# yixuan/spectra

Measured on AMD Instinct MI355X. Metric: eigenpairs_per_sec, higher is better.
Workload: dtype f64

## Files before the change

include/mispec.h:

```cpp
#ifndef MISPEC_H
#define MISPEC_H

#include <stdint.h>

#ifdef __cplusplus
extern "C" {
#endif

#define MISPEC_OK 0
#define MISPEC_EINVAL (-1)
#define MISPEC_ELOGIC (-2)
#define MISPEC_ERUNTIME (-3)

typedef struct mispec_ctx mispec_ctx;
typedef struct mispec_csr mispec_csr;
typedef struct mispec_fac mispec_fac;

const char* mispec_last_error(void);
const char* mispec_version(void);

int mispec_set_option(const char* name, const char* value);
const char* mispec_get_option(const char* name);

int mispec_ctx_create(int device, void* hip_stream, mispec_ctx** out);
// ... 32 lines not shown
int64_t mispec_csr_rows(const mispec_csr* A);
int64_t mispec_csr_cols(const mispec_csr* A);
int64_t mispec_csr_local_rows(const mispec_csr* A);
int64_t mispec_csr_local_nnz(const mispec_csr* A);
int mispec_csr_offset_codes(const mispec_csr* A);
int mispec_csr_use_offset_codes(mispec_csr* A, int enable);
int mispec_csr_use_windows(mispec_csr* A, int enable);
int mispec_csr_windows_info(const mispec_csr* A, int64_t* blocks, int64_t* covered_entries, int64_t* lds_doubles);
int mispec_csr_windows_in_use(const mispec_csr* A);
int mispec_csr_windows_table(const mispec_csr* A, int32_t* records_out, int64_t capacity);
int mispec_csr_windows_host(int64_t n_rows, int64_t n_cols, int64_t row_begin, const int32_t* rowptr, const int32_t* colind,
                            int32_t* records_out);
int mispec_csr_spmv_format(const mispec_csr* A);
int mispec_csr_set_spmv_format(mispec_csr* A, int format);
double mispec_csr_spmv_bytes(const mispec_csr* A, int stored);
int mispec_csr_coeff(const mispec_csr* A, int64_t i, int64_t j, double* out);
int mispec_csr_download(const mispec_csr* A, int32_t* rowptr_host, int32_t* colind_host, double* val_host);

int mispec_spmv(const mispec_csr* A, const double* x_dev, double* y_dev);
int mispec_spmv_host(const mispec_csr* A, const double* x_host, double* y_host);
int mispec_spmm_host(const mispec_csr* A, const double* X_host, int64_t ldx, int k, double* Y_host, int64_t ldy);
int mispec_spmm(const mispec_csr* A, const double* X_dev, int64_t ldx, int k, double* Y_dev, int64_t ldy);
int mispec_spmm_plan(int k, int forced_panel, int* widths_out, int cap, int* count);
int mispec_csr_reorder(mispec_csr* A, int method, int* applied);
int mispec_csr_reordering(const mispec_csr* A, double* far_before, double* far_after);
int mispec_csr_permutation(const mispec_csr* A, int32_t* perm_out);
int mispec_csr_tiles_info(const mispec_csr* A, int64_t* segments, int64_t* entries, int64_t* padding, int64_t* chunks);
int mispec_csr_staged_info(const mispec_csr* A, int64_t* bins, int64_t* slots, int64_t* batches, int64_t* chunks);
int mispec_last_ingest_info(double* seconds_out, int count);
int mispec_ingest_threads(void);
// ... 184 lines not shown
```

spectra_amd/__init__.py:

```python
import ctypes as C
import enum
import os

import numpy as np

from . import _capi
from ._capi import MispecError, Profile, build_library, check, lib

__all__ = ["SortRule", "CompInfo", "Context", "SparseSymMatProd", "SparseGenMatProd", "SparseSymShiftSolve", "SymEigsSolver",
           "SymEigsShiftSolver", "GenEigsSolver", "SVDMatOp", "PartialSVDSolver", "SparseRegularInverse", "SparseCholesky", "SymGEigsSolver", "SymShiftInvert", "SymGEigsShiftSolver", "SparseGenRealShiftSolve", "GenEigsRealShiftSolver", "shard_block",
           "Factorization", "tridiag_qr", "tridiag_eigen", "hess_qr", "double_shift_qr", "hess_schur", "hess_eigen", "MispecError", "build_library", "shard_range", "BAND_OFFSETS", "SYNTH_SEED",
           "SparseHermMatProd", "DenseHermMatProd", "HermEigsSolver", "spmm_plan"]

BAND_OFFSETS = (1, 2, 3, 1000, 1001, 100000, 100001)
SYNTH_SEED = 20240607


ORTH_MODES = {"reference": 0, "onesweep": 1, "onesweep-eager": 1 | 0x100, "onesweep-recorrect": 1 | 0x200, "onesweep-restart-check": 1 | 0x400,
              "onesweep-onered": 1 | 0x800, "onesweep-twored": 1 | 0x1000, "onesweep-onered-eager": 1 | 0x800 | 0x100}


def _orth_mode_value(mode):
    if isinstance(mode, str):
        if mode not in ORTH_MODES:
            raise ValueError("unknown orthogonalisation mode %r: one of %s" % (mode, ", ".join(sorted(ORTH_MODES))))
        return ORTH_MODES[mode]
    if isinstance(mode, int) and mode in ORTH_MODES.values():
# ... 165 lines not shown


def get_option(name):
    v = lib().mispec_get_option(name.encode())
    return None if v is None else v.decode()


def spmm_plan(k, panel=0):
    cap = max(int(k), 1)
    out = (C.c_int * cap)()
    count = C.c_int(0)
    check(lib().mispec_spmm_plan(int(k), int(panel), out, cap, C.byref(count)))
    return [out[i] for i in range(count.value)]


def default_context():
    global _default_ctx
    if _default_ctx is None:
        _default_ctx = Context(0)
    return _default_ctx


class _DeviceMatrix:

    def __init__(self, ctx, handle):
        self.ctx = ctx
        self.h = handle

    def rows(self):
        return lib().mispec_csr_rows(self.h)
# ... 49 lines not shown
        return 12.0 * self.nnz() + 4.0 * (self.local_rows() + 1) + 8.0 * self.cols() + 8.0 * self.local_rows()

    def offset_codes(self):
        return int(lib().mispec_csr_offset_codes(self.h))

    def use_offset_codes(self, enable=True):
        check(lib().mispec_csr_use_offset_codes(self.h, 1 if enable else 0))

    def use_windows(self, enable=True):
        check(lib().mispec_csr_use_windows(self.h, -1 if enable is None else (1 if enable else 0)))

    def windows_info(self):
        a, b, c = C.c_int64(0), C.c_int64(0), C.c_int64(0)
        check(lib().mispec_csr_windows_info(self.h, C.byref(a), C.byref(b), C.byref(c)))
        return {"blocks": a.value, "covered_entries": b.value, "lds_doubles": c.value}

    def windows_in_use(self):
        return bool(lib().mispec_csr_windows_in_use(self.h))

    def windows_table(self):
        nb = (self.local_rows() + 255) // 256
        out = np.empty((nb, 32), dtype=np.int32)
        check(lib().mispec_csr_windows_table(self.h, _ip(out), out.size))
        return out

    def spmv_format(self):
        return int(lib().mispec_csr_spmv_format(self.h))

    def set_spmv_format(self, fmt=-1):
        check(lib().mispec_csr_set_spmv_format(self.h, int(fmt)))
# ... 1401 lines not shown
```

spectra_amd/_capi.py:

```python
import ctypes as C
import os
import subprocess

_PKG = os.path.dirname(os.path.abspath(__file__))
LIB_PATH = os.path.join(_PKG, "libmispec.so")
EXTRAS_LIB_PATH = os.path.join(_PKG, "libmispec_extras.so")
EXTRAS_PREFIXES = ("mispec_davidson_", "mispec_zdense_", "mispec_zfac_", "mispec_zcsr_", "mispec_hermeigs_")
CSRC = os.path.join(_PKG, "csrc")

MISPEC_OK, MISPEC_EINVAL, MISPEC_ELOGIC, MISPEC_ERUNTIME = 0, -1, -2, -3


class MispecError(RuntimeError):
    """HIP / RCCL failure or a failed small decomposition (std::runtime_error in the C++ API)."""


def build_library(force=False, verbose=False):
    cmd = ["make", "-C", CSRC, "-j8"] + (["-B"] if force else [])
    out = subprocess.run(cmd, stdout=subprocess.PIPE, stderr=subprocess.STDOUT, text=True)
    if verbose or out.returncode != 0:
        print(out.stdout)
    if out.returncode != 0:
        raise RuntimeError("building libmispec.so failed")
    return LIB_PATH
# ... 51 lines not shown
    "mispec_csr_destroy": (C.c_int, [_vp]),
    "mispec_csr_rows": (C.c_int64, [_vp]),
    "mispec_csr_cols": (C.c_int64, [_vp]),
    "mispec_csr_local_rows": (C.c_int64, [_vp]),
    "mispec_csr_local_nnz": (C.c_int64, [_vp]),
    "mispec_csr_offset_codes": (C.c_int, [_vp]),
    "mispec_csr_use_offset_codes": (C.c_int, [_vp, C.c_int]),
    "mispec_csr_use_windows": (C.c_int, [_vp, C.c_int]),
    "mispec_csr_windows_info": (C.c_int, [_vp, _lp, _lp, _lp]),
    "mispec_csr_windows_table": (C.c_int, [_vp, _ip, C.c_int64]),
    "mispec_csr_windows_in_use": (C.c_int, [_vp]),
    "mispec_csr_windows_host": (C.c_int, [C.c_int64, C.c_int64, C.c_int64, _ip, _ip, _ip]),
    "mispec_csr_spmv_format": (C.c_int, [_vp]),
    "mispec_csr_set_spmv_format": (C.c_int, [_vp, C.c_int]),
    "mispec_csr_spmv_bytes": (C.c_double, [_vp, C.c_int]),
    "mispec_csr_coeff": (C.c_int, [_vp, C.c_int64, C.c_int64, _dp]),
    "mispec_csr_download": (C.c_int, [_vp, _ip, _ip, _dp]),
    "mispec_spmv": (C.c_int, [_vp, _vp, _vp]),
    "mispec_spmv_host": (C.c_int, [_vp, _dp, _dp]),
    "mispec_spmm_host": (C.c_int, [_vp, _dp, C.c_int64, C.c_int, _dp, C.c_int64]),
    "mispec_spmv_time": (C.c_int, [_vp, _vp, _vp, C.c_int, C.POINTER(C.c_float)]),
    "mispec_spmm": (C.c_int, [_vp, _vp, C.c_int64, C.c_int, _vp, C.c_int64]),
    "mispec_spmm_time": (C.c_int, [_vp, _vp, C.c_int64, C.c_int, _vp, C.c_int64, C.c_int, C.POINTER(C.c_float)]),
    "mispec_spmm_plan": (C.c_int, [C.c_int, C.c_int, C.POINTER(C.c_int), C.c_int, C.POINTER(C.c_int)]),
    "mispec_symshift_level_plan": (C.c_int, [C.c_int64, C.c_int64, C.c_int, _lp, _lp, _lp, _lp]),
    "mispec_symshift_create": (C.c_int, [_vp, C.c_int64, _ip, _ip, _dp, C.c_char, C.c_int, _vpp]),
    "mispec_symshift_destroy": (C.c_int, [_vp]),
    "mispec_symshift_rows": (C.c_int64, [_vp]),
    "mispec_symshift_bandwidth": (C.c_int, [_vp, _lp, _lp, C.POINTER(C.c_int)]),
    "mispec_csr_tiles_info": (C.c_int, [_vp, _lp, _lp, _lp, _lp]),
# ... 225 lines not shown
```

spectra_amd/csrc/common.hpp:

```cpp
#pragma once

#include <hip/hip_runtime.h>

#include <cstdint>
#include <cstdio>
#include <cstdlib>
#include <new>
#include <functional>
#include <utility>
#include <stdexcept>
#include <string>
#include <vector>

#include "../../include/mispec.h"
#include "../../include/mispec_extras.h"

namespace mispec {

struct Error : std::runtime_error
{
    int code;
    Error(int c, const std::string& m) : std::runtime_error(m), code(c) {}
};

// ... 96 lines not shown
    void alloc(size_t count)
    {
        if (p)
            (void) hipHostFree(p);
        p = nullptr;
        MISPEC_HIP(hipHostMalloc(reinterpret_cast<void**>(&p), count * sizeof(T), hipHostMallocDefault));
        n = count;
    }
};

inline int64_t round_up(int64_t x, int64_t m) { return (x + m - 1) / m * m; }

enum class Opt
{
    orth, one_reduction, orth_kernel, host_turn, small, restart_sync, host_steps, overlap, csr_win, spec_corr, exchange, reorder,
    spmv_staged, spmv_tiles, spmm, host_threads, shift, count
};
enum class Orth { onesweep, onesweep_eager, reference };
enum class OrthKernel { dma, dma2, reg, unset };
enum class HostTurn { fast, copy };
enum class Small { host, host_serial, device };
enum class Exchange { allgather, halo, unset };
enum class Reorder { automatic, rcm, none };
enum class Tri { automatic, off, on };
enum class Spmm { automatic, off, w2, w4, w8 };
int option_choice(Opt o);
template <typename E>
E option_choice(Opt o, E unset)
{
    const int i = option_choice(o);
    return i < 0 ? unset : E(i);
}
bool option_flag(Opt o, bool unset);
int option_int(Opt o, int unset);
struct ShiftOptions
{
    int lds = 1;
    int batch = 0;
    int lanes = 0;
// ... 65 lines not shown
```

spectra_amd/csrc/csr.hip:

```cpp
#include "csr_kernels.hpp"
#include "reorder.hpp"

#include <hip/hip_ext.h>

#include <chrono>

#include <algorithm>
#include <cstdlib>
#include <cstring>
#include <memory>
#include <numeric>

using namespace mispec;

namespace {

template <bool EPI, bool NT, int kThreads, bool CODES, int ITERS = 4>
__global__ __launch_bounds__(kThreads) void k_spmv_csr_stream(const int32_t* __restrict__ rowptr,
                                                               const int32_t* __restrict__ colind,
                                                               const double* __restrict__ val,
                                                               const double* __restrict__ x, double* __restrict__ y,
                                                               int64_t nrows, int nblocks, SpmvEpilogue epi, SpmvCodes cd)
{
    constexpr int kLoadIters = ITERS;
// ... 531 lines not shown
    std::vector<int32_t> rp, ci;
    std::vector<double> v;
    permute_csr(n, rowptr, colind, val, perm, rp, ci, v);
    std::unique_ptr<mispec_csr> B(upload_rows(A.ctx, n, n, rp.data(), ci.data(), v.data(), false, A.structurally_symmetric));
    A.rowptr.swap(B->rowptr);
    A.colind.swap(B->colind);
    A.val.swap(B->val);
    A.codes.swap(B->codes);
    A.dict.swap(B->dict);
    A.dia.swap(B->dia);
    A.dia_off.swap(B->dia_off);
    std::swap(A.ndict, B->ndict);
    std::swap(A.dia_ld, B->dia_ld);
    std::swap(A.ndia, B->ndia);
    std::swap(A.dia_win, B->dia_win);
    A.tiles.swap(B->tiles);
    A.staged.swap(B->staged);
    A.wtab.swap(B->wtab);
    std::swap(A.win_lds_doubles, B->win_lds_doubles);
    std::swap(A.win_covered, B->win_covered);
    std::swap(A.win_blocks, B->win_blocks);
    A.nnz = B->nnz;
    A.perm.alloc(size_t(n));
    MISPEC_HIP(hipMemcpy(A.perm.p, perm.data(), size_t(n) * sizeof(int32_t), hipMemcpyHostToDevice));
    A.perm_host.swap(perm);
    A.inv_host.swap(inv);
    A.reorder_method = 1;
    A.far_before = before;
    A.far_after = after;
    return true;
// ... 859 lines not shown
```

spectra_amd/csrc/csr.hpp:

```cpp
#pragma once
#include <vector>

#include "common.hpp"
#include "tiles.hpp"
#include "staged.hpp"

struct mispec_dia_windows
{
    int nc = 0;
    int total = 0;
    int start[8];
    int len[8];
    int base[8];
    int idx[32];
};

struct mispec_csr
{
    mispec_ctx* ctx = nullptr;
    int64_t n_rows = 0;
    int64_t n_cols = 0;
    int64_t row_begin = 0;
    int64_t row_end = 0;
    int64_t nnz = 0;
    mispec::DevBuf<int32_t> rowptr;
    mispec::DevBuf<int32_t> colind;
    mispec::DevBuf<double> val;
    mispec::DevBuf<uint8_t> codes;
    mispec::DevBuf<int32_t> dict;
    int ndict = 0;
    bool use_codes = true;
    mispec::DevBuf<double> dia;
    mispec::DevBuf<int32_t> dia_off;
    int64_t dia_ld = 0;
    int ndia = 0;
    mispec_dia_windows dia_win;
    mispec::DevBuf<int32_t> wtab;
    int win_lds_doubles = 0;
    int64_t win_covered = 0;
    int64_t win_blocks = 0;
    int use_windows = -1;
    bool windows_active() const
    {
        if (wtab.p == nullptr || win_lds_doubles <= 0 || use_windows == 0)
            return false;
        return use_windows == 1 || double(nnz) >= 9.0 * double(local_rows());
    }
    int forced_format = -1;
    mispec::DevTiles tiles;
    mispec::DevStaged staged;
    mispec::DevBuf<int32_t> perm;
// ... 3 lines not shown
    bool structurally_symmetric = false;
    mutable mispec::DevBuf<double> perm_x, perm_y;
    bool reordered() const { return perm.p != nullptr; }
    mutable mispec::DevBuf<double> stage_x, stage_y;
    mutable mispec::DevBuf<double> spmm_x;

    int64_t local_rows() const { return row_end - row_begin; }
    double algorithmic_bytes() const
    {
        return 12.0 * double(nnz) + 4.0 * double(local_rows() + 1) + 8.0 * double(n_cols) + 8.0 * double(local_rows());
    }
    int spmv_format() const;
    double stored_bytes_for(int format) const
    {
        if (format == 2)
            return 8.0 * double(ndia) * double(local_rows()) + 8.0 * double(n_cols) + 8.0 * double(local_rows());
        if (format == 4)
            return staged.stored_bytes(local_rows(), n_cols);
        if (format == 3)
            return 12.0 * double(tiles.entries) + 8.0 * double(tiles.nchunks) + 12.0 * double(tiles.nseg) + 8.0 * double(n_cols) +
                   8.0 * double(local_rows());
        const double per_entry = format == 1 ? 9.0 : 12.0;
        return per_entry * double(nnz) + 4.0 * double(local_rows() + 1) + 8.0 * double(n_cols) + 8.0 * double(local_rows());
    }
    double stored_bytes() const
    {
        return stored_bytes_for(spmv_format());
    }
};

namespace mispec {
// ... 36 lines not shown
```

spectra_amd/csrc/csr_dia.hip:

```cpp
#include "csr_kernels.hpp"

#include <algorithm>
#include <cstdlib>
#include <cstring>
#include <numeric>
#include <vector>

using namespace mispec;

namespace {

constexpr int kMaxDia = 32;
constexpr int kDiaGroup = 8;

__global__ __launch_bounds__(256) void k_build_dia(const int32_t* __restrict__ rowptr, const uint8_t* __restrict__ codes,
                                                   const double* __restrict__ val, const int32_t* __restrict__ pos_of_code,
                                                   int64_t nloc, int64_t ld, double* __restrict__ dia, int* __restrict__ bad, int nd_blocked)
{
    const int64_t r = int64_t(blockIdx.x) * 256 + threadIdx.x;
    if (r >= nloc)
        return;
    int last = -1;
    for (int p = rowptr[r]; p < rowptr[r + 1]; p++)
    {
        const int pos = pos_of_code[codes[p]];
        if (pos <= last)
            *bad = 1;
        last = pos;
        if (nd_blocked)
            dia[(int64_t(blockIdx.x) * nd_blocked + pos) * 256 + threadIdx.x] = val[p];
        else
            dia[int64_t(pos) * ld + r] = val[p];
    }
}

__device__ __forceinline__ double add_rounded_product(double acc, double a, double b)
{
#pragma clang fp contract(off)
    const double p = a * b;
    return acc + p;
}

struct DiaArgs
{
    const double* dia;
    const int32_t* off;
    int64_t ld;
    int nd;
    int col_max;
    int64_t row_begin;
};
__device__ __forceinline__ const double* dia_row(const DiaArgs& da, int lb, int t, int64_t& stride)
{
    if (da.ld == 0)
    {
        stride = 256;
        return da.dia + int64_t(lb) * da.nd * 256 + t;
    }
    stride = da.ld;
    return da.dia + int64_t(lb) * 256 + t;
}

template <bool EPI>
__global__ __launch_bounds__(256) void k_spmv_dia(DiaArgs da, const double* __restrict__ x, double* __restrict__ y, int64_t nrows,
                                                  int nblocks, SpmvEpilogue epi)
{
// ... 47 lines not shown
        }
        const double total = block_reduce_sum(contrib, red);
        if (tid == 0)
            epi.partials[lb] = total;
    }
    else if (tid < nr)
        y[row0 + tid] = acc;
}

template <bool EPI, int NG, int NCW = 8, bool POST = false>
__global__ __launch_bounds__(256) void k_spmv_dia_win(DiaArgs da, mispec_dia_windows w, const double* __restrict__ x,
                                                      double* __restrict__ y, int64_t nrows, int nblocks, SpmvEpilogue epi)
{
    extern __shared__ double xs[];
    __shared__ double red[4];
    const int per = (nblocks + 7) >> 3;
    const int lmap = (int(blockIdx.x) & 7) * per + (int(blockIdx.x) >> 3);
    if (lmap >= nblocks)
        return;
    const int lb = epi.first_block + lmap;
    if (EPI && epi.status && *epi.status != 0)
        return;
    const int tid = threadIdx.x;
    double beta = 1.0;
    if (POST)
    {
        StepState* st = static_cast<StepState*>(epi.post_scale_state);
        beta = st->beta;
        const bool first = (lmap == 0 && tid == 0);
        if (beta < epi.post_scale_eps_sqrt)
        {
            if (first)
            {
                st->status = kStepSmallBeta;
                st->stop_step = epi.post_scale_step;
                st->stop_count = 0;
            }
            return;
        }
        if (first)
            st->subd[epi.post_scale_step - 1] = beta;
    }
    const int64_t row0 = int64_t(lb) * 256;
    const int nr = int(min(int64_t(256), nrows - row0));
    int64_t vstride;
    const double* vrow = dia_row(da, lb, min(tid, nr - 1), vstride);
    double v[NG * kDiaGroup];
#pragma unroll
    for (int k = 0; k < NG * kDiaGroup; k++)
        v[k] = __builtin_nontemporal_load(vrow + int64_t(min(k, da.nd - 1)) * vstride);
    double vprev_early = 0.0, vrow_early = 0.0, hprev_early = 0.0;
    const bool early = EPI && tid < nr;
    if (early)
    {
        if (epi.v_prev)
        {
            vprev_early = epi.v_prev[row0 + tid];
            hprev_early = POST ? beta : (epi.h_prev_dev ? *epi.h_prev_dev : epi.h_prev);
        }
        vrow_early = epi.v_rows[row0 + tid];
        if (POST)
            vrow_early = vrow_early / beta;
    }
    const int64_t g0 = da.row_begin + row0;
    const auto xat = [&](int64_t col) { return x[min(max(col, int64_t(0)), int64_t(da.col_max))]; };
// ... 32 lines not shown
        for (int c = 0; c < w.nc; c++)
        {
            const int span = w.len[c] - 256;
            for (int t = tid + 256; t < before + span; t += 256)
                if (t >= before)
                {
                    const double xv = xat(g0 + w.start[c] + 256 + (t - before));
                    xs[w.base[c] + 256 + (t - before)] = xv;
                }
            before += span;
        }
    }
    __syncthreads();
    double acc = 0.0;
#pragma unroll
    for (int k = 0; k < NG * kDiaGroup; k++)
        if (k < da.nd)
            acc = add_rounded_product(acc, v[k], xs[w.idx[k] + tid]);
    if (EPI)
    {
        double contrib = 0.0;
        if (tid < nr)
        {
            const int64_t row = row0 + tid;
            double yv = POST ? acc / beta : acc;
            if (epi.v_prev)
                yv -= (early ? hprev_early : (epi.h_prev_dev ? *epi.h_prev_dev : epi.h_prev)) *
                      (early ? vprev_early : epi.v_prev[row]);
            y[row] = yv;
            contrib = (early ? vrow_early : epi.v_rows[row]) * yv;
        }
        const double total = block_reduce_sum(contrib, red);
        if (tid == 0)
            epi.partials[lb] = total;
    }
    else if (tid < nr)
        y[row0 + tid] = acc;
}

template <bool EPI, int NG, int NCW = 8, bool POST = false>
__global__ __launch_bounds__(128) void k_spmv_dia_win2(DiaArgs da, mispec_dia_windows w, const double* __restrict__ x,
                                                       double* __restrict__ y, int64_t nrows, int nblocks, SpmvEpilogue epi)
{
    extern __shared__ double xs[];
    __shared__ double red[4];
    const int per = (nblocks + 7) >> 3;
    const int lmap = (int(blockIdx.x) & 7) * per + (int(blockIdx.x) >> 3);
    if (lmap >= nblocks)
        return;
    const int lb = epi.first_block + lmap;
    if (EPI && epi.status && *epi.status != 0)
        return;
    const int tid = threadIdx.x;
    double beta = 1.0;
    if (POST)
    {
        StepState* st = static_cast<StepState*>(epi.post_scale_state);
        beta = st->beta;
        const bool first = (lmap == 0 && tid == 0);
        if (beta < epi.post_scale_eps_sqrt)
        {
            if (first)
            {
                st->status = kStepSmallBeta;
                st->stop_step = epi.post_scale_step;
                st->stop_count = 0;
            }
            return;
        }
        if (first)
            st->subd[epi.post_scale_step - 1] = beta;
    }
    const int64_t row0 = int64_t(lb) * 256;
    const int nr = int(min(int64_t(256), nrows - row0));
    const int r0 = 2 * tid;
    const double* vrow = da.dia + int64_t(lb) * da.nd * 256 + r0;
    double2 v[NG * kDiaGroup];
#pragma unroll
    for (int k = 0; k < NG * kDiaGroup; k++)
    {
        const v2d t2 = __builtin_nontemporal_load(reinterpret_cast<const v2d*>(vrow + int64_t(min(k, da.nd - 1)) * 256));
        v[k] = make_double2(t2.x, t2.y);
    }
    double2 vprev_e = make_double2(0.0, 0.0), vrow_e = make_double2(0.0, 0.0);
    double hprev_e = 0.0;
    const bool have0 = r0 < nr, have1 = r0 + 1 < nr;
    if (EPI && have0)
    {
        if (epi.v_prev)
        {
            if (have1)
                vprev_e = *reinterpret_cast<const double2*>(epi.v_prev + row0 + r0);
            else
                vprev_e.x = epi.v_prev[row0 + r0];
            hprev_e = POST ? beta : (epi.h_prev_dev ? *epi.h_prev_dev : epi.h_prev);
        }
        if (have1)
// ... 51 lines not shown
    if (tails > 256)
    {
        int before = 0;
        for (int c = 0; c < w.nc; c++)
        {
            const int span = w.len[c] - 256;
            for (int t = tid + 256; t < before + span; t += 128)
                if (t >= before)
                    xs[w.base[c] + 256 + (t - before)] = xat(g0 + w.start[c] + 256 + (t - before));
            before += span;
        }
    }
    __syncthreads();
    double acc0 = 0.0, acc1 = 0.0;
#pragma unroll
    for (int k = 0; k < NG * kDiaGroup; k++)
        if (k < da.nd)
        {
            acc0 = add_rounded_product(acc0, v[k].x, xs[w.idx[k] + r0]);
            acc1 = add_rounded_product(acc1, v[k].y, xs[w.idx[k] + r0 + 1]);
        }
    if (EPI)
    {
        double* cbuf = xs + w.total;
        double c0 = 0.0, c1 = 0.0;
        double2 yv;
        yv.x = POST ? acc0 / beta : acc0;
        yv.y = POST ? acc1 / beta : acc1;
        if (epi.v_prev)
        {
            yv.x -= hprev_e * vprev_e.x;
// ... 20 lines not shown
                red[k] = s;
        }
        __syncthreads();
        if (tid == 0)
            epi.partials[lb] = (red[0] + red[1]) + (red[2] + red[3]);
    }
    else
    {
        if (have1)
            *reinterpret_cast<double2*>(y + row0 + r0) = make_double2(acc0, acc1);
        else if (have0)
            y[row0 + r0] = acc0;
    }
}

}

namespace mispec {

void build_dia(mispec_csr& A, const std::vector<int32_t>& dict)
{
    const int64_t nloc = A.local_rows();
    const int nd = int(dict.size());
    if (nd == 0 || nd > kMaxDia || nloc == 0 || double(A.nnz) < 0.75 * double(nd) * double(nloc))
        return;
    std::vector<int32_t> order(static_cast<size_t>(nd)), pos(static_cast<size_t>(nd)), offs(static_cast<size_t>(nd));
    std::iota(order.begin(), order.end(), 0);
    std::sort(order.begin(), order.end(), [&](int32_t a, int32_t b) { return dict[size_t(a)] < dict[size_t(b)]; });
    for (int k = 0; k < nd; k++)
    {
// ... 37 lines not shown
            {
                ok = false;
                break;
            }
            const int c = w.nc++;
            w.start[c] = offs[size_t(first)];
            w.len[c] = 256 + (offs[size_t(k) - 1] - offs[size_t(first)]);
            w.base[c] = w.total;
            for (int d = first; d < k; d++)
                w.idx[d] = w.total + (offs[size_t(d)] - offs[size_t(first)]);
            w.total += w.len[c];
            first = k;
        }
    if (ok)
        A.dia_win = w;
}

void launch_spmv_dia(const mispec_csr& A, const SpmvLaunch& L)
{
    const dim3 grid = L.grid, block = L.block;
    const int64_t nloc = L.nloc;
    const int nblocks = L.nblocks;
    const SpmvEpilogue* epi = L.epi;
    const SpmvEpilogue e = L.e;
    const hipEvent_t ev_start = L.ev_start, ev_stop = L.ev_stop;
    const double* x_dev = L.x_dev;
    double* y_dev = L.y_dev;
        const DiaArgs da{A.dia.p, A.dia_off.p, A.dia_ld, A.ndia, int(A.n_cols - 1), A.row_begin};
        const bool dia2 = A.dia_win.nc > 0 && A.dia_ld == 0 && A.ndia <= 2 * kDiaGroup &&
                          (reinterpret_cast<uintptr_t>(y_dev) & 15) == 0 &&
                          (!epi || ((reinterpret_cast<uintptr_t>(e.v_rows) & 15) == 0 && (reinterpret_cast<uintptr_t>(e.v_prev) & 15) == 0));
        if (dia2)
        {
            const size_t lds2 = size_t(A.dia_win.total + 256) * sizeof(double);
            const dim3 block2(128);
            const int ng = (A.ndia + kDiaGroup - 1) / kDiaGroup;
            const bool post = epi && e.post_scale_state;
#define MISPEC_DIA2_LAUNCH(E, G, W, P)                                                                                                  \
    do                                                                                                                                  \
    {                                                                                                                                   \
        if (ev_start && ev_stop)                                                                                                        \
            hipExtLaunchKernelGGL((k_spmv_dia_win2<E, G, W, P>), grid, block2, lds2, A.ctx->stream, ev_start, ev_stop, 0, da, A.dia_win, \
                                  x_dev, y_dev, nloc, nblocks, e);                                                                      \
// ... 2 lines not shown
                               nblocks, e);                                                                                             \
    } while (0)
#define MISPEC_DIA2_W(E, G, P)               \
    do                                       \
    {                                        \
        if (A.dia_win.nc <= 4)               \
            MISPEC_DIA2_LAUNCH(E, G, 4, P);  \
        else if (A.dia_win.nc <= 6)          \
            MISPEC_DIA2_LAUNCH(E, G, 6, P);  \
        else                                 \
            MISPEC_DIA2_LAUNCH(E, G, 8, P);  \
    } while (0)
#define MISPEC_DIA2_G(E, P)          \
    do                               \
    {                                \
        if (ng == 1)                 \
            MISPEC_DIA2_W(E, 1, P);  \
        else                         \
            MISPEC_DIA2_W(E, 2, P);  \
    } while (0)
            if (post)
                MISPEC_DIA2_G(true, true);
            else if (epi)
                MISPEC_DIA2_G(true, false);
            else
                MISPEC_DIA2_G(false, false);
#undef MISPEC_DIA2_G
#undef MISPEC_DIA2_W
#undef MISPEC_DIA2_LAUNCH
            MISPEC_HIP(hipGetLastError());
            return;
        }
        if (A.dia_win.nc > 0)
        {
            const size_t lds = size_t(A.dia_win.total) * sizeof(double);
            const int ng = (A.ndia + kDiaGroup - 1) / kDiaGroup;
#define MISPEC_DIA_WIN_W(E, G, W)                                                                                             \
    do                                                                                                                     \
    {                                                                                                                      \
        if (ev_start && ev_stop)                                                                                           \
            hipExtLaunchKernelGGL((k_spmv_dia_win<E, G, W>), grid, block, lds, A.ctx->stream, ev_start, ev_stop, 0, da, A.dia_win, x_dev, \
                                  y_dev, nloc, nblocks, e);                                                                \
        else                                                                                                               \
            hipLaunchKernelGGL((k_spmv_dia_win<E, G, W>), grid, block, lds, A.ctx->stream, da, A.dia_win, x_dev, y_dev, nloc, nblocks, e); \
    } while (0)
#define MISPEC_DIA_WIN(E, G)              \
    do                                    \
    {                                     \
        if (A.dia_win.nc <= 4)            \
            MISPEC_DIA_WIN_W(E, G, 4);    \
        else if (A.dia_win.nc <= 6)       \
            MISPEC_DIA_WIN_W(E, G, 6);    \
        else                              \
            MISPEC_DIA_WIN_W(E, G, 8);    \
    } while (0)
#define MISPEC_DIA_WIN_G(E)          \
    do                               \
    {                                \
        if (ng == 1)                 \
            MISPEC_DIA_WIN(E, 1);    \
        else if (ng == 2)            \
            MISPEC_DIA_WIN(E, 2);    \
        else if (ng == 3)            \
            MISPEC_DIA_WIN(E, 3);    \
        else                         \
            MISPEC_DIA_WIN(E, 4);    \
    } while (0)
            if (epi && e.post_scale_state)
            {
#define MISPEC_DIA_WIN_POST_W(G, W)                                                                                                    \
    do                                                                                                                                 \
    {                                                                                                                                  \
        if (ev_start && ev_stop)                                                                                                       \
            hipExtLaunchKernelGGL((k_spmv_dia_win<true, G, W, true>), grid, block, lds, A.ctx->stream, ev_start, ev_stop, 0, da, A.dia_win, \
                                  x_dev, y_dev, nloc, nblocks, e);                                                                     \
        else                                                                                                                           \
            hipLaunchKernelGGL((k_spmv_dia_win<true, G, W, true>), grid, block, lds, A.ctx->stream, da, A.dia_win, x_dev, y_dev, nloc, \
                               nblocks, e);                                                                                            \
    } while (0)
#define MISPEC_DIA_WIN_POST(G)               \
    do                                       \
    {                                        \
        if (A.dia_win.nc <= 4)               \
            MISPEC_DIA_WIN_POST_W(G, 4);     \
        else if (A.dia_win.nc <= 6)          \
            MISPEC_DIA_WIN_POST_W(G, 6);     \
        else                                 \
            MISPEC_DIA_WIN_POST_W(G, 8);     \
    } while (0)
                if (ng == 1)
                    MISPEC_DIA_WIN_POST(1);
                else if (ng == 2)
                    MISPEC_DIA_WIN_POST(2);
                else if (ng == 3)
                    MISPEC_DIA_WIN_POST(3);
                else
                    MISPEC_DIA_WIN_POST(4);
#undef MISPEC_DIA_WIN_POST
#undef MISPEC_DIA_WIN_POST_W
            }
            else if (epi)
                MISPEC_DIA_WIN_G(true);
            else
                MISPEC_DIA_WIN_G(false);
#undef MISPEC_DIA_WIN_G
#undef MISPEC_DIA_WIN
#undef MISPEC_DIA_WIN_W
            MISPEC_HIP(hipGetLastError());
            return;
        }
        if (ev_start && ev_stop)
        {
// ... 15 lines not shown
```

spectra_amd/csrc/ctx.hip:

```cpp
#include "common.hpp"

#include <dlfcn.h>
#include <rccl/rccl.h>

#include <algorithm>
#include <condition_variable>
#include <exception>
#include <thread>
#include <cstring>
#include <mutex>

namespace mispec {
static thread_local std::string g_last_error;
void set_last_error(const std::string& msg) { g_last_error = msg; }

void* big_host_alloc(size_t bytes)
{
    void* q = std::malloc(bytes ? bytes : 1);
    if (!q)
        throw std::bad_alloc();
    return q;
}

namespace {
// ... 24 lines not shown
    {Opt::restart_sync, "restart_sync", "MISPEC_RESTART_SYNC", Kind::choice, {"0", "1"}, 0, 0, "synchronising fused restart"},
    {Opt::host_steps, "host_steps", "MISPEC_HOST_STEPS", Kind::choice, {"0", "1"}, 0, 0, "host-synchronous steps"},
    {Opt::overlap, "overlap", "MISPEC_OVERLAP", Kind::choice, {"0", "1"}, 0, 0,
     "sharded product: overlap of the exchange with the local rows (default 1)"},
    {Opt::csr_win, "csr_win", "MISPEC_CSR_WIN", Kind::choice, {"0", "1"}, 0, 0, "x windows of the int32 CSR kernel (default 1)"},
    {Opt::spec_corr, "spec_corr", "MISPEC_SPEC_CORR", Kind::integer, {}, 1, 4,
     "corrections enqueued speculatively per step (unset: 2, 1 when sharded)"},
    {Opt::exchange, "exchange", "MISPEC_EXCHANGE", Kind::choice, {"allgather", "halo"}, 0, 0,
     "sharded product: the all-gather or the neighbour exchange (unset: the exchange when the halos are small)"},
    {Opt::reorder, "reorder", "MISPEC_REORDER", Kind::choice, {"auto", "rcm", "none"}, 0, 0,
     "reverse Cuthill-McKee ordering at ingest and of the shift solve"},
    {Opt::spmv_staged, "spmv_staged", "MISPEC_SPMV_STAGED", Kind::choice, {"auto", "0", "1"}, 0, 0, "staged SpMV format"},
    {Opt::spmv_tiles, "spmv_tiles", "MISPEC_SPMV_TILES", Kind::choice, {"auto", "0", "1"}, 0, 0, "column-blocked tile SpMV format"},
    {Opt::spmm, "spmm", "MISPEC_SPMM", Kind::choice, {"auto", "0", "2", "4", "8"}, 0, 0,
     "widest panel of a block product (0: one SpMV per column)"},
    {Opt::host_threads, "host_threads", "MISPEC_HOST_THREADS", Kind::integer, {}, 1, kMaxInt,
     "upper bound on the host threads of the ingest and of the shift solve's host-side factorisation"},
    {Opt::shift, "shift", "MISPEC_SHIFT", Kind::shift, {}, 0, 0, "kernel variants of the banded shift solve"},
};
static_assert(sizeof(kOptions) / sizeof(kOptions[0]) == size_t(Opt::count), "one entry per option");
constexpr bool entries_in_order()
{
    for (size_t i = 0; i < size_t(Opt::count); i++)
        if (kOptions[i].id != Opt(i))
            return false;
    return true;
}
static_assert(entries_in_order(), "kOptions is indexed by Opt");

struct ShiftKey
// ... 617 lines not shown
```

Before: 21.18.

## Store only upper diagonals of symmetric DIA matrices and read mirrored partners

At DIA build time, each lower diagonal whose mirrored upper diagonal holds bit-identical values is detected on the device. The matrix is then repacked so those lower diagonals are not stored, and the SpMV kernels get template variants that read each such diagonal from its upper partner at a shifted row offset. This cuts the diagonal value bytes streamed per product roughly in half for symmetric banded matrices. The cost is extra build-time checking and compaction, lead padding blocks, more kernel instantiations, and partner reads that may be unaligned or hit cache differently when the shift is odd or far.

```diff
diff --git a/include/mispec.h b/include/mispec.h
--- a/include/mispec.h
+++ b/include/mispec.h
@@ -70,6 +70,8 @@
 int mispec_csr_spmv_format(const mispec_csr* A);
 int mispec_csr_set_spmv_format(mispec_csr* A, int format);
 double mispec_csr_spmv_bytes(const mispec_csr* A, int stored);
+int mispec_csr_dia_info(const mispec_csr* A, int* ndia, int* nstored, int* nmirrored, int* lead_blocks);
+int mispec_dia_sym_plan(const int32_t* offsets, int nd, int64_t reach, int32_t* out_flags, int* lead_blocks);
 int mispec_csr_coeff(const mispec_csr* A, int64_t i, int64_t j, double* out);
 int mispec_csr_download(const mispec_csr* A, int32_t* rowptr_host, int32_t* colind_host, double* val_host);
 
diff --git a/spectra_amd/__init__.py b/spectra_amd/__init__.py
--- a/spectra_amd/__init__.py
+++ b/spectra_amd/__init__.py
@@ -10,7 +10,7 @@
 __all__ = ["SortRule", "CompInfo", "Context", "SparseSymMatProd", "SparseGenMatProd", "SparseSymShiftSolve", "SymEigsSolver",
            "SymEigsShiftSolver", "GenEigsSolver", "SVDMatOp", "PartialSVDSolver", "SparseRegularInverse", "SparseCholesky", "SymGEigsSolver", "SymShiftInvert", "SymGEigsShiftSolver", "SparseGenRealShiftSolve", "GenEigsRealShiftSolver", "shard_block",
            "Factorization", "tridiag_qr", "tridiag_eigen", "hess_qr", "double_shift_qr", "hess_schur", "hess_eigen", "MispecError", "build_library", "shard_range", "BAND_OFFSETS", "SYNTH_SEED",
-           "SparseHermMatProd", "DenseHermMatProd", "HermEigsSolver", "spmm_plan"]
+           "SparseHermMatProd", "DenseHermMatProd", "HermEigsSolver", "spmm_plan", "dia_sym_plan"]
 
 BAND_OFFSETS = (1, 2, 3, 1000, 1001, 100000, 100001)
 SYNTH_SEED = 20240607
@@ -206,6 +206,14 @@
     return [out[i] for i in range(count.value)]
 
 
+def dia_sym_plan(offsets, reach=-1):
+    offs = np.ascontiguousarray(offsets, dtype=np.int32)
+    flags = np.zeros(offs.size, dtype=np.int32)
+    lead = C.c_int(0)
+    check(lib().mispec_dia_sym_plan(_ip(offs), int(offs.size), int(reach), _ip(flags), C.byref(lead)))
+    return [bool(f) for f in flags], lead.value
+
+
 def default_context():
     global _default_ctx
     if _default_ctx is None:
@@ -285,6 +293,11 @@
         a, b, c = C.c_int64(0), C.c_int64(0), C.c_int64(0)
         check(lib().mispec_csr_windows_info(self.h, C.byref(a), C.byref(b), C.byref(c)))
         return {"blocks": a.value, "covered_entries": b.value, "lds_doubles": c.value}
+
+    def dia_info(self):
+        a, b, c, d = C.c_int(0), C.c_int(0), C.c_int(0), C.c_int(0)
+        check(lib().mispec_csr_dia_info(self.h, C.byref(a), C.byref(b), C.byref(c), C.byref(d)))
+        return {"ndia": a.value, "nstored": b.value, "nmirrored": c.value, "lead_blocks": d.value}
 
     def windows_in_use(self):
         return bool(lib().mispec_csr_windows_in_use(self.h))
diff --git a/spectra_amd/_capi.py b/spectra_amd/_capi.py
--- a/spectra_amd/_capi.py
+++ b/spectra_amd/_capi.py
@@ -89,6 +89,8 @@
     "mispec_csr_spmv_format": (C.c_int, [_vp]),
     "mispec_csr_set_spmv_format": (C.c_int, [_vp, C.c_int]),
     "mispec_csr_spmv_bytes": (C.c_double, [_vp, C.c_int]),
+    "mispec_csr_dia_info": (C.c_int, [_vp, C.POINTER(C.c_int), C.POINTER(C.c_int), C.POINTER(C.c_int), C.POINTER(C.c_int)]),
+    "mispec_dia_sym_plan": (C.c_int, [_ip, C.c_int, C.c_int64, _ip, C.POINTER(C.c_int)]),
     "mispec_csr_coeff": (C.c_int, [_vp, C.c_int64, C.c_int64, _dp]),
     "mispec_csr_download": (C.c_int, [_vp, _ip, _ip, _dp]),
     "mispec_spmv": (C.c_int, [_vp, _vp, _vp]),
diff --git a/spectra_amd/csrc/common.hpp b/spectra_amd/csrc/common.hpp
--- a/spectra_amd/csrc/common.hpp
+++ b/spectra_amd/csrc/common.hpp
@@ -134,7 +134,7 @@
 enum class Opt
 {
     orth, one_reduction, orth_kernel, host_turn, small, restart_sync, host_steps, overlap, csr_win, spec_corr, exchange, reorder,
-    spmv_staged, spmv_tiles, spmm, host_threads, shift, count
+    spmv_staged, spmv_tiles, spmm, dia_sym, host_threads, shift, count
 };
 enum class Orth { onesweep, onesweep_eager, reference };
 enum class OrthKernel { dma, dma2, reg, unset };
@@ -143,6 +143,7 @@
 enum class Exchange { allgather, halo, unset };
 enum class Reorder { automatic, rcm, none };
 enum class Tri { automatic, off, on };
+enum class DiaSym { automatic, off, all };
 enum class Spmm { automatic, off, w2, w4, w8 };
 int option_choice(Opt o);
 template <typename E>
diff --git a/spectra_amd/csrc/csr.hip b/spectra_amd/csrc/csr.hip
--- a/spectra_amd/csrc/csr.hip
+++ b/spectra_amd/csrc/csr.hip
@@ -569,6 +569,7 @@
     std::swap(A.dia_ld, B->dia_ld);
     std::swap(A.ndia, B->ndia);
     std::swap(A.dia_win, B->dia_win);
+    std::swap(A.dia_plan, B->dia_plan);
     A.tiles.swap(B->tiles);
     A.staged.swap(B->staged);
     A.wtab.swap(B->wtab);
diff --git a/spectra_amd/csrc/csr.hpp b/spectra_amd/csrc/csr.hpp
--- a/spectra_amd/csrc/csr.hpp
+++ b/spectra_amd/csrc/csr.hpp
@@ -13,6 +13,16 @@
     int len[8];
     int base[8];
     int idx[32];
+};
+
+struct mispec_dia_plan
+{
+    int nstored = 0;
+    int lead = 0;
+    int src[32];
+    int shift[32];
+    static constexpr int kStream = 256;
+    constexpr int slot(int k) const { return src[k] & (kStream - 1); }
 };
 
 struct mispec_csr
@@ -35,6 +45,7 @@
     int64_t dia_ld = 0;
     int ndia = 0;
     mispec_dia_windows dia_win;
+    mispec_dia_plan dia_plan;
     mispec::DevBuf<int32_t> wtab;
     int win_lds_doubles = 0;
     int64_t win_covered = 0;
@@ -68,7 +79,8 @@
     double stored_bytes_for(int format) const
     {
         if (format == 2)
-            return 8.0 * double(ndia) * double(local_rows()) + 8.0 * double(n_cols) + 8.0 * double(local_rows());
+            return 8.0 * double(dia_plan.nstored) * double(local_rows() + 256 * int64_t(dia_plan.lead)) + 8.0 * double(n_cols) +
+                   8.0 * double(local_rows());
         if (format == 4)
             return staged.stored_bytes(local_rows(), n_cols);
         if (format == 3)
diff --git a/spectra_amd/csrc/csr_dia.hip b/spectra_amd/csrc/csr_dia.hip
--- a/spectra_amd/csrc/csr_dia.hip
+++ b/spectra_amd/csrc/csr_dia.hip
@@ -12,6 +12,9 @@
 
 constexpr int kMaxDia = 32;
 constexpr int kDiaGroup = 8;
+constexpr int64_t kDiaSymReach = 131072;
+constexpr bool kMirrorNontemporal = false;
+constexpr int kDiaMir = 8;
 
 __global__ __launch_bounds__(256) void k_build_dia(const int32_t* __restrict__ rowptr, const uint8_t* __restrict__ codes,
                                                    const double* __restrict__ val, const int32_t* __restrict__ pos_of_code,
@@ -34,6 +37,51 @@
     }
 }
 
+struct DiaPairs
+{
+    int count = 0;
+    int lo[kMaxDia / 2], hi[kMaxDia / 2], k[kMaxDia / 2];
+};
+__global__ __launch_bounds__(256) void k_dia_sym_check(const double* __restrict__ full, int nd, int64_t nloc, DiaPairs pairs,
+                                                       int* __restrict__ bad)
+{
+    const int64_t r = int64_t(blockIdx.x) * 256 + threadIdx.x;
+    if (r >= nloc)
+        return;
+    const unsigned long long* bits = reinterpret_cast<const unsigned long long*>(full);
+    for (int p = 0; p < pairs.count; p++)
+    {
+        const int64_t s = r - pairs.k[p];
+        if (s < 0)
+            continue;
+        const unsigned long long a = bits[(int64_t(blockIdx.x) * nd + pairs.lo[p]) * 256 + threadIdx.x];
+        const unsigned long long b = bits[((s >> 8) * nd + pairs.hi[p]) * 256 + (s & 255)];
+        if (a != b)
+            bad[p] = 1;
+    }
+}
+__global__ __launch_bounds__(256) void k_dia_compact(const double* __restrict__ full, int nd, int64_t nloc, mispec_dia_plan plan,
+                                                     double* __restrict__ out)
+{
+    const int64_t lb = blockIdx.x;
+    const int t = threadIdx.x;
+    const double* src = full + lb * nd * 256 + t;
+    double* dst = out + (lb + plan.lead) * plan.nstored * 256 + t;
+    const int64_t r = lb * 256 + t;
+    for (int k = 0; k < nd; k++)
+    {
+        const double a = src[int64_t(k) * 256];
+        const int sh = plan.shift[k];
+        if (sh == 0)
+            dst[int64_t(plan.slot(k)) * 256] = a;
+        else if (r < sh && r < nloc)
+        {
+            const int64_t e = int64_t(plan.lead) * 256 + r - sh;
+            out[((e >> 8) * plan.nstored + plan.slot(k)) * 256 + (e & 255)] = a;
+        }
+    }
+}
+
 __device__ __forceinline__ double add_rounded_product(double acc, double a, double b)
 {
 #pragma clang fp contract(off)
@@ -49,7 +97,46 @@
     int nd;
     int col_max;
     int64_t row_begin;
+    mispec_dia_plan plan;
 };
+template <int N>
+struct PlanRegs
+{
+    int src[N], shift[N];
+    __device__ __forceinline__ explicit PlanRegs(const mispec_dia_plan& pl)
+    {
+#pragma unroll
+        for (int k = 0; k < N; k++)
+        {
+            src[k] = pl.src[k];
+            shift[k] = pl.shift[k];
+        }
+    }
+};
+__device__ __forceinline__ const double* dia_src(const DiaArgs& da, int src, int64_t e)
+{
+    return da.dia + ((e >> 8) * da.plan.nstored + (src & (mispec_dia_plan::kStream - 1))) * 256 + (e & 255);
+}
+__device__ __forceinline__ double dia_load1(const DiaArgs& da, int src, int shift, int64_t e)
+{
+    const double* q = dia_src(da, src, e - shift);
+    return (src & mispec_dia_plan::kStream) ? __builtin_nontemporal_load(q) : *q;
+}
+__device__ __forceinline__ double2 dia_load2(const DiaArgs& da, int src, int shift, int64_t e)
+{
+    const bool nt = (src & mispec_dia_plan::kStream) != 0;
+    if (shift & 1)
+    {
+        const double* q0 = dia_src(da, src, e - shift);
+        const double* q1 = dia_src(da, src, e - shift + 1);
+        if (nt)
+            return make_double2(__builtin_nontemporal_load(q0), __builtin_nontemporal_load(q1));
+        return make_double2(*q0, *q1);
+    }
+    const v2d* q = reinterpret_cast<const v2d*>(dia_src(da, src, e - shift));
+    const v2d t2 = nt ? __builtin_nontemporal_load(q) : *q;
+    return make_double2(t2.x, t2.y);
+}
 __device__ __forceinline__ const double* dia_row(const DiaArgs& da, int lb, int t, int64_t& stride)
 {
     if (da.ld == 0)
@@ -127,6 +214,9 @@
 {
     extern __shared__ double xs[];
     __shared__ double red[4];
+    constexpr bool MIR = NG >= kDiaMir;
+    constexpr int NV = (NG % kDiaMir) * kDiaGroup;
+    const PlanRegs<MIR ? NV : 1> pl(da.plan);
     const int per = (nblocks + 7) >> 3;
     const int lmap = (int(blockIdx.x) & 7) * per + (int(blockIdx.x) >> 3);
     if (lmap >= nblocks)
@@ -156,12 +246,22 @@
     }
     const int64_t row0 = int64_t(lb) * 256;
     const int nr = int(min(int64_t(256), nrows - row0));
-    int64_t vstride;
-    const double* vrow = dia_row(da, lb, min(tid, nr - 1), vstride);
-    double v[NG * kDiaGroup];
-#pragma unroll
-    for (int k = 0; k < NG * kDiaGroup; k++)
-        v[k] = __builtin_nontemporal_load(vrow + int64_t(min(k, da.nd - 1)) * vstride);
+    double v[NV];
+    if constexpr (MIR)
+    {
+        const int64_t erow = (int64_t(da.plan.lead) + lb) * 256 + min(tid, nr - 1);
+#pragma unroll
+        for (int k = 0; k < NV; k++)
+            v[k] = dia_load1(da, pl.src[k], pl.shift[k], erow);
+    }
+    else
+    {
+        int64_t vstride;
+        const double* vrow = dia_row(da, lb, min(tid, nr - 1), vstride);
+#pragma unroll
+        for (int k = 0; k < NV; k++)
+            v[k] = __builtin_nontemporal_load(vrow + int64_t(min(k, da.nd - 1)) * vstride);
+    }
     double vprev_early = 0.0, vrow_early = 0.0, hprev_early = 0.0;
     const bool early = EPI && tid < nr;
     if (early)
@@ -224,7 +324,7 @@
     __syncthreads();
     double acc = 0.0;
 #pragma unroll
-    for (int k = 0; k < NG * kDiaGroup; k++)
+    for (int k = 0; k < NV; k++)
         if (k < da.nd)
             acc = add_rounded_product(acc, v[k], xs[w.idx[k] + tid]);
     if (EPI)
@@ -254,6 +354,9 @@
 {
     extern __shared__ double xs[];
     __shared__ double red[4];
+    constexpr bool MIR = NG >= kDiaMir;
+    constexpr int NV = (NG % kDiaMir) * kDiaGroup;
+    const PlanRegs<MIR ? NV : 1> pl(da.plan);
     const int per = (nblocks + 7) >> 3;
     const int lmap = (int(blockIdx.x) & 7) * per + (int(blockIdx.x) >> 3);
     if (lmap >= nblocks)
@@ -284,13 +387,23 @@
     const int64_t row0 = int64_t(lb) * 256;
     const int nr = int(min(int64_t(256), nrows - row0));
     const int r0 = 2 * tid;
-    const double* vrow = da.dia + int64_t(lb) * da.nd * 256 + r0;
-    double2 v[NG * kDiaGroup];
-#pragma unroll
-    for (int k = 0; k < NG * kDiaGroup; k++)
-    {
-        const v2d t2 = __builtin_nontemporal_load(reinterpret_cast<const v2d*>(vrow + int64_t(min(k, da.nd - 1)) * 256));
-        v[k] = make_double2(t2.x, t2.y);
+    double2 v[NV];
+    if constexpr (MIR)
+    {
+        const int64_t erow = (int64_t(da.plan.lead) + lb) * 256 + r0;
+#pragma unroll
+        for (int k = 0; k < NV; k++)
+            v[k] = dia_load2(da, pl.src[k], pl.shift[k], erow);
+    }
+    else
+    {
+        const double* vrow = da.dia + int64_t(lb) * da.nd * 256 + r0;
+#pragma unroll
+        for (int k = 0; k < NV; k++)
+        {
+            const v2d t2 = __builtin_nontemporal_load(reinterpret_cast<const v2d*>(vrow + int64_t(min(k, da.nd - 1)) * 256));
+            v[k] = make_double2(t2.x, t2.y);
+        }
     }
     double2 vprev_e = make_double2(0.0, 0.0), vrow_e = make_double2(0.0, 0.0);
     double hprev_e = 0.0;
@@ -372,7 +485,7 @@
     __syncthreads();
     double acc0 = 0.0, acc1 = 0.0;
 #pragma unroll
-    for (int k = 0; k < NG * kDiaGroup; k++)
+    for (int k = 0; k < NV; k++)
         if (k < da.nd)
         {
             acc0 = add_rounded_product(acc0, v[k].x, xs[w.idx[k] + r0]);
@@ -423,6 +536,78 @@
     }
 }
 
+int dia_sym_rule(const int32_t* offs, int nd, int64_t reach, int32_t* flags)
+{
+    int64_t kmax = 0;
+    for (int i = 0; i < nd; i++)
+    {
+        flags[i] = 0;
+        const int64_t k = -int64_t(offs[i]);
+        if (k <= 0 || (reach >= 0 && k > reach))
+            continue;
+        for (int j = 0; j < nd; j++)
+            if (int64_t(offs[j]) == k)
+                flags[i] = 1;
+        if (flags[i])
+            kmax = std::max(kmax, k);
+    }
+    return int((kmax + 255) / 256);
+}
+
+mispec_dia_plan make_plan(const int32_t* offs, int nd, const int32_t* mirrored)
+{
+    mispec_dia_plan pl;
+    int64_t kmax = 0;
+    for (int i = 0; i < nd; i++)
+    {
+        pl.shift[i] = mirrored[i] ? -offs[i] : 0;
+        if (!mirrored[i])
+            pl.src[i] = pl.nstored++ + mispec_dia_plan::kStream;
+        else
+            kmax = std::max<int64_t>(kmax, -int64_t(offs[i]));
+    }
+    pl.lead = int((kmax + 255) / 256);
+    for (int i = 0; i < nd; i++)
+        if (mirrored[i])
+            for (int j = 0; j < nd; j++)
+                if (offs[j] == -offs[i])
+                {
+                    pl.src[j] = pl.slot(j);
+                    pl.src[i] = pl.slot(j) + (kMirrorNontemporal ? mispec_dia_plan::kStream : 0);
+                }
+    for (int i = nd; i < 32; i++)
+    {
+        pl.src[i] = pl.src[nd - 1];
+        pl.shift[i] = pl.shift[nd - 1];
+    }
+    return pl;
+}
+
+}
+
+extern "C" int mispec_dia_sym_plan(const int32_t* offsets, int nd, int64_t reach, int32_t* out_flags, int* lead_blocks)
+{
+    return guarded([&] {
+        MISPEC_REQUIRE(nd >= 0 && nd <= kMaxDia && (nd == 0 || (offsets && out_flags)), "mispec_dia_sym_plan: bad argument");
+        const int lead = dia_sym_rule(offsets, nd, reach, out_flags);
+        if (lead_blocks)
+            *lead_blocks = lead;
+    });
+}
+
+extern "C" int mispec_csr_dia_info(const mispec_csr* A, int* ndia, int* nstored, int* nmirrored, int* lead_blocks)
+{
+    return guarded([&] {
+        MISPEC_REQUIRE(A, "mispec_csr_dia_info: NULL argument");
+        if (ndia)
+            *ndia = A->ndia;
+        if (nstored)
+            *nstored = A->ndia ? A->dia_plan.nstored : 0;
+        if (nmirrored)
+            *nmirrored = A->ndia ? A->ndia - A->dia_plan.nstored : 0;
+        if (lead_blocks)
+            *lead_blocks = A->ndia ? A->dia_plan.lead : 0;
+    });
 }
 
 namespace mispec {
@@ -490,6 +675,53 @@
         }
     if (ok)
         A.dia_win = w;
+    const std::vector<int32_t> none(static_cast<size_t>(nd), 0);
+    A.dia_plan = make_plan(offs.data(), nd, none.data());
+    const DiaSym sym = option_choice(Opt::dia_sym, DiaSym::automatic);
+    if (!ok || sym == DiaSym::off)
+        return;
+    std::vector<int32_t> flags(static_cast<size_t>(nd), 0);
+    dia_sym_rule(offs.data(), nd, sym == DiaSym::all ? int64_t(-1) : kDiaSymReach, flags.data());
+    DiaPairs pairs;
+    int which[kMaxDia / 2];
+    for (int i = 0; i < nd; i++)
+        if (flags[size_t(i)])
+        {
+            const int p = pairs.count++;
+            which[p] = i;
+            pairs.lo[p] = i;
+            pairs.hi[p] = int(std::find(offs.begin(), offs.end(), -offs[size_t(i)]) - offs.begin());
+            pairs.k[p] = -offs[size_t(i)];
+        }
+    if (pairs.count == 0)
+        return;
+    DevBuf<int> d_asym;
+    d_asym.alloc(size_t(pairs.count));
+    MISPEC_HIP(hipMemsetAsync(d_asym.p, 0, size_t(pairs.count) * sizeof(int), st));
+    const unsigned nblk = unsigned(ld / 256);
+    hipLaunchKernelGGL(k_dia_sym_check, dim3(nblk), dim3(256), 0, st, A.dia.p, nd, nloc, pairs, d_asym.p);
+    MISPEC_HIP(hipGetLastError());
+    int asym[kMaxDia / 2] = {};
+    MISPEC_HIP(hipMemcpyAsync(asym, d_asym.p, size_t(pairs.count) * sizeof(int), hipMemcpyDeviceToHost, st));
+    MISPEC_HIP(hipStreamSynchronize(st));
+    int nmir = 0;
+    for (int p = 0; p < pairs.count; p++)
+    {
+        if (asym[p])
+            flags[size_t(which[p])] = 0;
+        nmir += flags[size_t(which[p])];
+    }
+    if (nmir == 0)
+        return;
+    const mispec_dia_plan plan = make_plan(offs.data(), nd, flags.data());
+    DevBuf<double> packed;
+    packed.alloc(size_t(ld + 256 * int64_t(plan.lead)) * size_t(plan.nstored));
+    MISPEC_HIP(hipMemsetAsync(packed.p, 0, packed.n * sizeof(double), st));
+    hipLaunchKernelGGL(k_dia_compact, dim3(nblk), dim3(256), 0, st, A.dia.p, nd, nloc, plan, packed.p);
+    MISPEC_HIP(hipGetLastError());
+    MISPEC_HIP(hipStreamSynchronize(st));
+    A.dia.swap(packed);
+    A.dia_plan = plan;
 }
 
 void launch_spmv_dia(const mispec_csr& A, const SpmvLaunch& L)
@@ -502,7 +734,9 @@
     const hipEvent_t ev_start = L.ev_start, ev_stop = L.ev_stop;
     const double* x_dev = L.x_dev;
     double* y_dev = L.y_dev;
-        const DiaArgs da{A.dia.p, A.dia_off.p, A.dia_ld, A.ndia, int(A.n_cols - 1), A.row_begin};
+        const DiaArgs da{A.dia.p, A.dia_off.p, A.dia_ld, A.ndia, int(A.n_cols - 1), A.row_begin, A.dia_plan};
+        const bool mir = A.dia_plan.nstored != A.ndia;
+        MISPEC_REQUIRE(!mir || (A.dia_ld == 0 && A.dia_win.nc > 0), "diagonal storage: a mirror plan needs the block layout and x windows");
         const bool dia2 = A.dia_win.nc > 0 && A.dia_ld == 0 && A.ndia <= 2 * kDiaGroup &&
                           (reinterpret_cast<uintptr_t>(y_dev) & 15) == 0 &&
                           (!epi || ((reinterpret_cast<uintptr_t>(e.v_rows) & 15) == 0 && (reinterpret_cast<uintptr_t>(e.v_prev) & 15) == 0));
@@ -535,10 +769,14 @@
 #define MISPEC_DIA2_G(E, P)          \
     do                               \
     {                                \
-        if (ng == 1)                 \
-            MISPEC_DIA2_W(E, 1, P);  \
-        else                         \
-            MISPEC_DIA2_W(E, 2, P);  \
+        if (ng == 1 && !mir)                   \
+            MISPEC_DIA2_W(E, 1, P);            \
+        else if (!mir)                         \
+            MISPEC_DIA2_W(E, 2, P);            \
+        else if (ng == 1)                      \
+            MISPEC_DIA2_W(E, kDiaMir + 1, P);  \
+        else                                   \
+            MISPEC_DIA2_W(E, kDiaMir + 2, P);  \
     } while (0)
             if (post)
                 MISPEC_DIA2_G(true, true);
@@ -555,7 +793,7 @@
         if (A.dia_win.nc > 0)
         {
             const size_t lds = size_t(A.dia_win.total) * sizeof(double);
-            const int ng = (A.ndia + kDiaGroup - 1) / kDiaGroup;
+            const int ng = (A.ndia + kDiaGroup - 1) / kDiaGroup + (mir ? kDiaMir : 0);
 #define MISPEC_DIA_WIN_W(E, G, W)                                                                                             \
     do                                                                                                                     \
     {                                                                                                                      \
@@ -578,14 +816,22 @@
 #define MISPEC_DIA_WIN_G(E)          \
     do                               \
     {                                \
-        if (ng == 1)                 \
-            MISPEC_DIA_WIN(E, 1);    \
-        else if (ng == 2)            \
-            MISPEC_DIA_WIN(E, 2);    \
-        else if (ng == 3)            \
-            MISPEC_DIA_WIN(E, 3);    \
-        else                         \
-            MISPEC_DIA_WIN(E, 4);    \
+        if (ng == 1)                           \
+            MISPEC_DIA_WIN(E, 1);              \
+        else if (ng == 2)                      \
+            MISPEC_DIA_WIN(E, 2);              \
+        else if (ng == 3)                      \
+            MISPEC_DIA_WIN(E, 3);              \
+        else if (ng == 4)                      \
+            MISPEC_DIA_WIN(E, 4);              \
+        else if (ng == kDiaMir + 1)            \
+            MISPEC_DIA_WIN(E, kDiaMir + 1);    \
+        else if (ng == kDiaMir + 2)            \
+            MISPEC_DIA_WIN(E, kDiaMir + 2);    \
+        else if (ng == kDiaMir + 3)            \
+            MISPEC_DIA_WIN(E, kDiaMir + 3);    \
+        else                                   \
+            MISPEC_DIA_WIN(E, kDiaMir + 4);    \
     } while (0)
             if (epi && e.post_scale_state)
             {
@@ -615,8 +861,16 @@
                     MISPEC_DIA_WIN_POST(2);
                 else if (ng == 3)
                     MISPEC_DIA_WIN_POST(3);
+                else if (ng == 4)
+                    MISPEC_DIA_WIN_POST(4);
+                else if (ng == kDiaMir + 1)
+                    MISPEC_DIA_WIN_POST(kDiaMir + 1);
+                else if (ng == kDiaMir + 2)
+                    MISPEC_DIA_WIN_POST(kDiaMir + 2);
+                else if (ng == kDiaMir + 3)
+                    MISPEC_DIA_WIN_POST(kDiaMir + 3);
                 else
-                    MISPEC_DIA_WIN_POST(4);
+                    MISPEC_DIA_WIN_POST(kDiaMir + 4);
 #undef MISPEC_DIA_WIN_POST
 #undef MISPEC_DIA_WIN_POST_W
             }
diff --git a/spectra_amd/csrc/ctx.hip b/spectra_amd/csrc/ctx.hip
--- a/spectra_amd/csrc/ctx.hip
+++ b/spectra_amd/csrc/ctx.hip
@@ -62,6 +62,8 @@
     {Opt::spmv_tiles, "spmv_tiles", "MISPEC_SPMV_TILES", Kind::choice, {"auto", "0", "1"}, 0, 0, "column-blocked tile SpMV format"},
     {Opt::spmm, "spmm", "MISPEC_SPMM", Kind::choice, {"auto", "0", "2", "4", "8"}, 0, 0,
      "widest panel of a block product (0: one SpMV per column)"},
+    {Opt::dia_sym, "dia_sym", "MISPEC_DIA_SYM", Kind::choice, {"auto", "0", "all"}, 0, 0,
+     "diagonal storage: lower diagonals read from their mirrored upper partner (auto: those within reach, 0: none, all)"},
     {Opt::host_threads, "host_threads", "MISPEC_HOST_THREADS", Kind::integer, {}, 1, kMaxInt,
      "upper bound on the host threads of the ingest and of the shift solve's host-side factorisation"},
     {Opt::shift, "shift", "MISPEC_SHIFT", Kind::shift, {}, 0, 0, "kernel variants of the banded shift solve"},
```

After: 22.63, median of 6. +6.8%, better.
